# coollabsio/maxio

Hardware: AMD Instinct MI355X
Metric: device-resident RS encode+reconstruct GiB/s (k+m, chunk_size); % HBM roofline (higher is better)
Workload: dtype u8

## Files before the change

maxio_amd/csrc/rs_kernel.hip:

```cpp
#include "kernels.hpp"

#include <cstdlib>

namespace mxec {
namespace {

constexpr int kThreads = 256;
constexpr int fast_vecs(uint32_t r) { return r <= 4 ? 4 : 2; }
constexpr uint64_t kEdgeTile = kThreads * 16;

struct Vec4 {
    uint32_t w[4];
};

__device__ __forceinline__ Vec4 load16(const uint8_t* p) {
    const uint4 v = *reinterpret_cast<const uint4*>(p);
    return Vec4{{v.x, v.y, v.z, v.w}};
}

__device__ __forceinline__ void store16(uint8_t* p, const uint32_t (&w)[4]) {
    *reinterpret_cast<uint4*>(p) = make_uint4(w[0], w[1], w[2], w[3]);
}

__device__ __forceinline__ Vec4 load_partial(const uint8_t* p, int64_t valid, bool aligned) {
    if (aligned && valid >= 16) return load16(p);
    Vec4 r{{0, 0, 0, 0}};
    for (int b = 0; b < 16; ++b)
        if (b < valid) r.w[b >> 2] |= uint32_t(p[b]) << (8 * (b & 3));
    return r;
}

__device__ __forceinline__ void store_partial(uint8_t* p, const uint32_t (&w)[4], int64_t valid,
                                              bool aligned) {
    if (aligned && valid >= 16) {
        store16(p, w);
        return;
    }
    for (int b = 0; b < 16; ++b)
        if (b < valid) p[b] = uint8_t(w[b >> 2] >> (8 * (b & 3)));
}

template <int R>
__device__ __forceinline__ void mac_dword(uint32_t (&acc)[R], uint32_t x, const uint32_t* __restrict__ t,
                                          const uint32_t (&hi)[R][2]) {
    const uint32_t s0 = x & 0x07070707u;
    const uint32_t s1 = (x >> 3) & 0x07070707u;
    const uint32_t s2 = (x >> 6) & 0x03030303u;
#pragma unroll
    for (int i = 0; i < R; ++i) {
        const uint32_t p0 = __builtin_amdgcn_perm(hi[i][0], t[8 * i + 0], s0);
        const uint32_t p1 = __builtin_amdgcn_perm(hi[i][1], t[8 * i + 2], s1);
        const uint32_t p2 = __builtin_amdgcn_perm(s2, t[8 * i + 4], s2);
        acc[i] = __builtin_amdgcn_bitop3_b32(acc[i], p0, p1, 0x96) ^ p2;
    }
}

template <int R, int V>
__device__ __forceinline__ void mac_column(uint32_t (&acc)[V][4][R], const Vec4 (&x)[V],
                                           const uint32_t* __restrict__ t) {
    uint32_t hi[R][2];
#pragma unroll
    for (int i = 0; i < R; ++i) {
        hi[i][0] = __builtin_amdgcn_readfirstlane(t[8 * i + 1]);
        hi[i][1] = __builtin_amdgcn_readfirstlane(t[8 * i + 3]);
        asm volatile("" : "+v"(hi[i][0]), "+v"(hi[i][1]));
    }
#pragma unroll
    for (int v = 0; v < V; ++v)
#pragma unroll
        for (int w = 0; w < 4; ++w) mac_dword<R>(acc[v][w], x[v].w[w], t, hi);
}

template <int R, int V>
__device__ __forceinline__ void mac_column_pair(uint32_t (&acc)[V][4][R], const Vec4 (&xa)[V], const Vec4 (&xb)[V],
                                                const uint32_t* __restrict__ ta, const uint32_t* __restrict__ tb) {
    uint32_t ha[R][2], hb[R][2];
#pragma unroll
    for (int i = 0; i < R; ++i) {
        ha[i][0] = __builtin_amdgcn_readfirstlane(ta[8 * i + 1]);
        ha[i][1] = __builtin_amdgcn_readfirstlane(ta[8 * i + 3]);
        hb[i][0] = __builtin_amdgcn_readfirstlane(tb[8 * i + 1]);
        hb[i][1] = __builtin_amdgcn_readfirstlane(tb[8 * i + 3]);
        asm volatile("" : "+v"(ha[i][0]), "+v"(ha[i][1]), "+v"(hb[i][0]), "+v"(hb[i][1]));
    }
#pragma unroll
    for (int v = 0; v < V; ++v)
#pragma unroll
        for (int w = 0; w < 4; ++w) {
            const uint32_t a = xa[v].w[w], b = xb[v].w[w];
            const uint32_t a0 = a & 0x07070707u, a1 = (a >> 3) & 0x07070707u, a2 = (a >> 6) & 0x03030303u;
            const uint32_t b0 = b & 0x07070707u, b1 = (b >> 3) & 0x07070707u, b2 = (b >> 6) & 0x03030303u;
#pragma unroll
            for (int i = 0; i < R; ++i) {
                const uint32_t pa0 = __builtin_amdgcn_perm(ha[i][0], ta[8 * i + 0], a0);
                const uint32_t pa1 = __builtin_amdgcn_perm(ha[i][1], ta[8 * i + 2], a1);
                const uint32_t pa2 = __builtin_amdgcn_perm(a2, ta[8 * i + 4], a2);
                const uint32_t pb0 = __builtin_amdgcn_perm(hb[i][0], tb[8 * i + 0], b0);
                const uint32_t pb1 = __builtin_amdgcn_perm(hb[i][1], tb[8 * i + 2], b1);
                const uint32_t pb2 = __builtin_amdgcn_perm(b2, tb[8 * i + 4], b2);
                uint32_t t = __builtin_amdgcn_bitop3_b32(acc[v][w][i], pa0, pa1, 0x96);
                t = __builtin_amdgcn_bitop3_b32(t, pa2, pb0, 0x96);
                acc[v][w][i] = __builtin_amdgcn_bitop3_b32(t, pb1, pb2, 0x96);
            }
        }
}

typedef const uint8_t __attribute__((address_space(1)))* gcptr;
typedef uint8_t __attribute__((address_space(1)))* gptr;

typedef uint32_t u32x4 __attribute__((ext_vector_type(4)));

__device__ __forceinline__ Vec4 gload16(gcptr p) {
    const u32x4 v = __builtin_nontemporal_load((const u32x4 __attribute__((address_space(1)))*)(p));
    return Vec4{{v.x, v.y, v.z, v.w}};
}
__device__ __forceinline__ Vec4 gload16_plain(gcptr p) {
    const u32x4 v = *(const u32x4 __attribute__((address_space(1)))*)(p);
    return Vec4{{v.x, v.y, v.z, v.w}};
}
__device__ __forceinline__ void gstore16(gptr p, const uint32_t (&w)[4]) {
    u32x4 v = {w[0], w[1], w[2], w[3]};
    __builtin_nontemporal_store(v, (u32x4 __attribute__((address_space(1)))*)(p));
}

__device__ __forceinline__ Vec4 mask_tail(Vec4 x, int32_t valid) {
#pragma unroll
    for (int w = 0; w < 4; ++w) {
        const int32_t nb = valid - 4 * w;
        const uint32_t mk = nb >= 4 ? 0xFFFFFFFFu : (nb <= 0 ? 0u : (0xFFFFFFFFu >> (32 - 8 * nb)));
        x.w[w] &= mk;
    }
    return x;
}

__device__ __forceinline__ uint32_t any_bits(const uint32_t (&d)[4]) { return d[0] | d[1] | d[2] | d[3]; }

__device__ __forceinline__ void report_first_bad(uint64_t* const* __restrict__ fbp, uint32_t row,
                                                 const uint32_t (&d)[4], uint64_t off) {
    const uint64_t bad = __builtin_amdgcn_ballot_w64(any_bits(d) != 0);
    if (bad == 0) return;
    if ((threadIdx.x & 63u) != uint32_t(__builtin_ctzll(bad))) return;
    const uint32_t w = d[0] ? 0u : d[1] ? 1u : d[2] ? 2u : 3u;
    const uint32_t x = d[0] ? d[0] : d[1] ? d[1] : d[2] ? d[2] : d[3];
    const uint64_t at = off + 4 * w + (uint32_t(__builtin_ctz(x)) >> 3);
    atomicMin(reinterpret_cast<unsigned long long*>(*fbp + row), static_cast<unsigned long long>(at));
}

enum : int { kStore = 0, kCmp = 1, kLocate = 2, kSeed = 3 };

struct LocArgs {
    LocateRec* const* rec = nullptr;
    const uint8_t* field = nullptr;
    const uint8_t* tab = nullptr;
    const uint32_t* off = nullptr;
};

struct LocTally {
    uint32_t first = ~0u;
    uint32_t n = 0;
    uint32_t cmin = ~0u, cmax = 0;
};

template <int R>
__device__ __forceinline__ void locate_dword(LocTally& t, const uint32_t (&d)[R], uint32_t rel, uint64_t col0,
                                             const uint8_t* __restrict__ field, const uint8_t* __restrict__ tab,
                                             const uint64_t* __restrict__ il, uint32_t k) {
    uint32_t any = 0;
#pragma unroll
    for (int i = 0; i < R; ++i) any |= d[i];
    if (any == 0) return;
#pragma unroll 1
    for (uint32_t b = 0; b < 4; ++b) {
        uint32_t s[R], nz = 0;
#pragma unroll
        for (int i = 0; i < R; ++i) {
            s[i] = (d[i] >> (8 * b)) & 0xFFu;
            nz += s[i] != 0;
        }
        if (nz == 0) continue;
        uint32_t c = kLocateNoShard;
        if (nz == 1) {
#pragma unroll
            for (int i = 0; i < R; ++i) c = s[i] ? k + uint32_t(i) : c;
        } else if (nz == uint32_t(R)) {
            if constexpr (R >= 2) {
                const uint32_t l0 = field[s[0]];
                uint32_t dl = uint32_t(field[s[1]]) + 255u - l0;
                dl = dl >= 255u ? dl - 255u : dl;
                const uint32_t j = tab[field[256 + dl]];
                if (j < k) {
                    bool ok = col0 + b < il[j];
#pragma unroll
                    for (int i = 2; i < R; ++i) {
                        uint32_t di = uint32_t(field[s[i]]) + 255u - l0;
                        di = di >= 255u ? di - 255u : di;
                        ok = ok && di == tab[256 * (1 + i) + j];
                    }
                    c = ok ? j : c;
                }
            }
        }
        t.n += 1;
        t.first = min(t.first, rel + b);
        t.cmin = min(t.cmin, c);
        t.cmax = max(t.cmax, c);
    }
}

__device__ __forceinline__ void locate_commit(LocateRec* rec, LocTally t, uint64_t base) {
#pragma unroll
    for (int o = 32; o > 0; o >>= 1) {
        t.first = min(t.first, uint32_t(__shfl_xor(t.first, o)));
        t.n += uint32_t(__shfl_xor(t.n, o));
        t.cmin = min(t.cmin, uint32_t(__shfl_xor(t.cmin, o)));
        t.cmax = max(t.cmax, uint32_t(__shfl_xor(t.cmax, o)));
    }
    if ((threadIdx.x & 63u) != 0 || t.n == 0) return;
    atomicMin(reinterpret_cast<unsigned long long*>(&rec->first_bad), static_cast<unsigned long long>(base + t.first));
    atomicAdd(reinterpret_cast<unsigned long long*>(&rec->n_bad), static_cast<unsigned long long>(t.n));
    atomicMin(&rec->shard_min, t.cmin);
    atomicMax(&rec->shard_max, t.cmax);
}

__global__ void rs_locate_init(LocateRec* __restrict__ recs, uint64_t n) {
    const uint64_t i = uint64_t(blockIdx.x) * blockDim.x + threadIdx.x;
    if (i < n) recs[i] = LocateRec{~uint64_t(0), 0, ~0u, 0};
}

template <int R, int POL = kStore>
__device__ __forceinline__ void edge_step(
    const uint8_t* const* __restrict__ in_ptrs, uint8_t* const* __restrict__ out_ptrs,
    const uint64_t* __restrict__ in_len, const uint64_t* __restrict__ out_len,
    const uint32_t* __restrict__ coef, const uint32_t* __restrict__ coef_off, uint64_t shard_size,
    uint32_t k, uint32_t r_total, uint32_t row0, const uint64_t* __restrict__ edge_list,
    uint32_t steps_per_tile, uint64_t tile_bytes, uint32_t aligned, uint64_t step,
    uint64_t* const* __restrict__ fb_ptrs = nullptr, LocArgs loc = {},
    const uint8_t* const* __restrict__ seed_ptrs = nullptr) {
    const uint64_t e = edge_list[step / steps_per_tile];
    const uint32_t obj = uint32_t(e >> 32);
    const uint64_t col = uint64_t(uint32_t(e)) * tile_bytes + (step % steps_per_tile) * kEdgeTile +
                         threadIdx.x * 16;
    if constexpr (POL == kLocate) {
        if (__builtin_amdgcn_ballot_w64(col < shard_size) == 0) return;
    } else {
        if (col >= shard_size) return;
    }
    const uint32_t* __restrict__ tab = coef + coef_off[obj] + row0 * 8;
    uint32_t acc[1][4][R];
    if constexpr (POL == kSeed) {
#pragma unroll
        for (int i = 0; i < R; ++i) {
            uint64_t olen = out_len[uint64_t(obj) * r_total + row0 + i];
            if (olen > shard_size) olen = shard_size;
            const int64_t valid = col < olen ? int64_t(olen - col) : 0;
            Vec4 sd{{0, 0, 0, 0}};
            if (valid > 0) sd = load_partial(seed_ptrs[uint64_t(obj) * r_total + row0 + i] + col, valid, aligned != 0);
#pragma unroll
            for (int w = 0; w < 4; ++w) acc[0][w][i] = sd.w[w];
        }
    } else {
#pragma unroll
        for (int w = 0; w < 4; ++w)
#pragma unroll
            for (int i = 0; i < R; ++i) acc[0][w][i] = 0;
    }
    const uint8_t* safe = reinterpret_cast<const uint8_t*>(coef);
    auto issue = [&](uint32_t j, Vec4& x, const uint8_t*& p, int64_t& valid) {
        const uint64_t len = in_len[uint64_t(obj) * k + j];
        valid = col < len ? int64_t(len - col) : 0;
        p = in_ptrs[uint64_t(obj) * k + j] + col;
        const bool full = aligned && valid >= 16;
        x = gload16_plain(gcptr(full ? p : safe));
    };
    auto fixup = [&](Vec4& x, const uint8_t* p, int64_t valid) {
        const bool full = aligned && valid >= 16;
#pragma unroll
        for (int w = 0; w < 4; ++w) x.w[w] = full ? x.w[w] : 0u;
        if (valid > 0 && !full) x = load_partial(p, valid, aligned != 0);
    };
    uint32_t j = 0;
    for (; j + 4 <= k; j += 4) {
        Vec4 x[4][1];
        const uint8_t* p[4];
        int64_t valid[4];
#pragma unroll
        for (int u = 0; u < 4; ++u) issue(j + u, x[u][0], p[u], valid[u]);
#pragma unroll
        for (int u = 0; u < 4; ++u) fixup(x[u][0], p[u], valid[u]);
#pragma unroll
        for (int u = 0; u < 4; ++u) mac_column<R, 1>(acc, x[u], tab + (j + u) * r_total * 8);
    }
    for (; j < k; ++j) {
        Vec4 x[1];
        const uint8_t* p;
        int64_t valid;
        issue(j, x[0], p, valid);
        fixup(x[0], p, valid);
        mac_column<R, 1>(acc, x, tab + j * r_total * 8);
    }
    if constexpr (POL == kLocate) {
        uint32_t df[4][R], any = 0;
#pragma unroll
        for (int i = 0; i < R; ++i) {
            uint64_t olen = out_len[uint64_t(obj) * r_total + row0 + i];
            if (olen > shard_size) olen = shard_size;
            const int64_t valid = col < olen ? int64_t(olen - col) : 0;
            Vec4 st{{0, 0, 0, 0}};
            if (valid > 0) st = load_partial(out_ptrs[uint64_t(obj) * r_total + row0 + i] + col, valid, aligned != 0);
            Vec4 d{{acc[0][0][i] ^ st.w[0], acc[0][1][i] ^ st.w[1], acc[0][2][i] ^ st.w[2], acc[0][3][i] ^ st.w[3]}};
            d = mask_tail(d, valid >= 16 ? 16 : int32_t(valid));
#pragma unroll
            for (int w = 0; w < 4; ++w) {
                df[w][i] = d.w[w];
                any |= d.w[w];
            }
        }
        if (__builtin_amdgcn_ballot_w64(any != 0) == 0) return;
        LocTally t;
        const uint8_t* __restrict__ ktab = loc.tab + loc.off[obj];
#pragma unroll
        for (int w = 0; w < 4; ++w)
            locate_dword<R>(t, df[w], threadIdx.x * 16 + 4 * w, col + 4 * w, loc.field, ktab,
                            in_len + uint64_t(obj) * k, k);
        locate_commit(loc.rec[obj], t, col - threadIdx.x * 16);
        return;
    }
    constexpr bool CMP = POL == kCmp;
#pragma unroll
    for (int i = 0; i < R; ++i) {
        uint64_t olen = out_len[uint64_t(obj) * r_total + row0 + i];
        if (olen > shard_size) olen = shard_size;
        if constexpr (CMP) {
            const int64_t valid = col < olen ? int64_t(olen - col) : 0;
            Vec4 st{{0, 0, 0, 0}};
            if (valid > 0) st = load_partial(out_ptrs[uint64_t(obj) * r_total + row0 + i] + col, valid, aligned != 0);
            Vec4 df{{acc[0][0][i] ^ st.w[0], acc[0][1][i] ^ st.w[1], acc[0][2][i] ^ st.w[2], acc[0][3][i] ^ st.w[3]}};
            df = mask_tail(df, valid >= 16 ? 16 : int32_t(valid));
            report_first_bad(fb_ptrs + obj, row0 + i, df.w, col);
        } else if (col < olen) {
            uint32_t o[4] = {acc[0][0][i], acc[0][1][i], acc[0][2][i], acc[0][3][i]};
            store_partial(out_ptrs[uint64_t(obj) * r_total + row0 + i] + col, o, int64_t(olen - col),
                          aligned != 0);
        }
    }
}

template <int R>
__global__ __launch_bounds__(kThreads) void rs_apply_edge(
    const uint8_t* const* __restrict__ in_ptrs, uint8_t* const* __restrict__ out_ptrs,
    const uint64_t* __restrict__ in_len, const uint64_t* __restrict__ out_len,
    const uint32_t* __restrict__ coef, const uint32_t* __restrict__ coef_off, uint64_t shard_size,
    uint32_t k, uint32_t r_total, uint32_t row0, const uint64_t* __restrict__ edge_list,
    uint32_t steps_per_tile, uint64_t tile_bytes, uint32_t aligned, uint64_t n_steps) {
    for (uint64_t step = blockIdx.x; step < n_steps; step += gridDim.x)
        edge_step<R>(in_ptrs, out_ptrs, in_len, out_len, coef, coef_off, shard_size, k, r_total, row0, edge_list,
                     steps_per_tile, tile_bytes, aligned, step);
}

template <int R>
__global__ __launch_bounds__(kThreads) void rs_verify_edge(
    const uint8_t* const* __restrict__ in_ptrs, uint8_t* const* __restrict__ out_ptrs,
    const uint64_t* __restrict__ in_len, const uint64_t* __restrict__ out_len,
    const uint32_t* __restrict__ coef, const uint32_t* __restrict__ coef_off, uint64_t shard_size,
    uint32_t k, uint32_t r_total, uint32_t row0, const uint64_t* __restrict__ edge_list,
    uint32_t steps_per_tile, uint64_t tile_bytes, uint32_t aligned, uint64_t n_steps,
    uint64_t* const* __restrict__ fb_ptrs) {
    for (uint64_t step = blockIdx.x; step < n_steps; step += gridDim.x)
        edge_step<R, kCmp>(in_ptrs, out_ptrs, in_len, out_len, coef, coef_off, shard_size, k, r_total, row0,
                           edge_list, steps_per_tile, tile_bytes, aligned, step, fb_ptrs);
}

template <int R>
__global__ __launch_bounds__(kThreads) void rs_update_edge(
    const uint8_t* const* __restrict__ in_ptrs, uint8_t* const* __restrict__ out_ptrs,
    const uint64_t* __restrict__ in_len, const uint64_t* __restrict__ out_len,
    const uint32_t* __restrict__ coef, const uint32_t* __restrict__ coef_off, uint64_t shard_size,
    uint32_t k, uint32_t r_total, uint32_t row0, const uint64_t* __restrict__ edge_list,
    uint32_t steps_per_tile, uint64_t tile_bytes, uint32_t aligned, uint64_t n_steps,
    const uint8_t* const* __restrict__ seed_ptrs) {
    for (uint64_t step = blockIdx.x; step < n_steps; step += gridDim.x)
        edge_step<R, kSeed>(in_ptrs, out_ptrs, in_len, out_len, coef, coef_off, shard_size, k, r_total, row0,
                            edge_list, steps_per_tile, tile_bytes, aligned, step, nullptr, {}, seed_ptrs);
}

template <int R>
__global__ __launch_bounds__(kThreads) void rs_locate_edge(
    const uint8_t* const* __restrict__ in_ptrs, uint8_t* const* __restrict__ out_ptrs,
    const uint64_t* __restrict__ in_len, const uint64_t* __restrict__ out_len,
    const uint32_t* __restrict__ coef, const uint32_t* __restrict__ coef_off, uint64_t shard_size,
    uint32_t k, uint32_t r_total, uint32_t row0, const uint64_t* __restrict__ edge_list,
    uint32_t steps_per_tile, uint64_t tile_bytes, uint32_t aligned, uint64_t n_steps, LocArgs loc) {
    for (uint64_t step = blockIdx.x; step < n_steps; step += gridDim.x)
        edge_step<R, kLocate>(in_ptrs, out_ptrs, in_len, out_len, coef, coef_off, shard_size, k, r_total, row0,
                              edge_list, steps_per_tile, tile_bytes, aligned, step, nullptr, loc);
}

__device__ __forceinline__ Vec4 gload16_upto(gcptr p, int32_t valid, gcptr safe) {
    return mask_tail(gload16(valid > 0 ? p : safe), valid);
}

template <int R, int V, int POL = kStore>
__device__ __forceinline__ void rs_tile(const uint8_t* const* __restrict__ ip, const uint64_t* __restrict__ il,
                                        uint8_t* const* __restrict__ op, const uint64_t* __restrict__ ol,
                                        const uint32_t* __restrict__ tab, uint32_t k, uint32_t stride,
                                        uint64_t base, gcptr safe, uint64_t* const* __restrict__ fbp = nullptr,
                                        uint32_t row = 0, LocArgs loc = {},
                                        const uint8_t* const* __restrict__ sp = nullptr) {
    constexpr bool CMP = POL == kCmp || POL == kLocate;
    constexpr uint32_t kTile = kThreads * 16 * V;
    const uint64_t end = base + kTile;
    const uint64_t lane = base + threadIdx.x * 16;
    const int32_t lane_off = int32_t(threadIdx.x * 16);

    uint32_t acc[V][4][R];
    if constexpr (POL == kSeed) {
#pragma unroll
        for (int i = 0; i < R; ++i) {
            const uint64_t olen = ol[i];
            gcptr q = ((gcptr)(sp[i])) + lane;
            Vec4 sd[V];
            if (olen >= end) {
#pragma unroll
                for (int v = 0; v < V; ++v) sd[v] = gload16(q + v * kThreads * 16);
            } else if (olen <= base) {
#pragma unroll
                for (int v = 0; v < V; ++v) sd[v] = Vec4{{0, 0, 0, 0}};
            } else {
                const int32_t d = int32_t(olen - base) - lane_off;
#pragma unroll
                for (int v = 0; v < V; ++v)
                    sd[v] = gload16_upto(q + v * kThreads * 16, d - v * int32_t(kThreads * 16), safe);
            }
#pragma unroll
            for (int v = 0; v < V; ++v)
#pragma unroll
                for (int w = 0; w < 4; ++w) acc[v][w][i] = sd[v].w[w];
        }
    } else {
#pragma unroll
        for (int v = 0; v < V; ++v)
#pragma unroll
            for (int w = 0; w < 4; ++w)
#pragma unroll
                for (int i = 0; i < R; ++i) acc[v][w][i] = 0;
    }

    auto load_in = [&](uint32_t jj, Vec4 (&x)[V]) {
        const uint64_t len = il[jj];
        gcptr p = ((gcptr)(ip[jj])) + lane;
        if (len >= end) {
#pragma unroll
            for (int v = 0; v < V; ++v) x[v] = gload16(p + v * kThreads * 16);
        } else if (len <= base) {
#pragma unroll
            for (int v = 0; v < V; ++v) x[v] = Vec4{{0, 0, 0, 0}};
        } else {
            const int32_t d = int32_t(len - base) - lane_off;
#pragma unroll
            for (int v = 0; v < V; ++v)
                x[v] = gload16_upto(p + v * kThreads * 16, d - v * int32_t(kThreads * 16), safe);
        }
    };

    uint32_t j = 0;
    for (; j + 4 <= k; j += 4) {
        Vec4 x[4][V];
        if (il[j] >= end && il[j + 1] >= end && il[j + 2] >= end && il[j + 3] >= end) {
#pragma unroll
            for (int jj = 0; jj < 4; ++jj) {
                gcptr p = ((gcptr)(ip[j + jj])) + lane;
#pragma unroll
                for (int v = 0; v < V; ++v) x[jj][v] = gload16(p + v * kThreads * 16);
            }
        } else {
#pragma unroll
            for (int jj = 0; jj < 4; ++jj) load_in(j + jj, x[jj]);
        }
        if constexpr (R >= 3) {
            mac_column_pair<R, V>(acc, x[0], x[1], tab + (j + 0) * stride * 8, tab + (j + 1) * stride * 8);
            mac_column_pair<R, V>(acc, x[2], x[3], tab + (j + 2) * stride * 8, tab + (j + 3) * stride * 8);
        } else {
#pragma unroll
            for (int jj = 0; jj < 4; ++jj) mac_column<R, V>(acc, x[jj], tab + (j + jj) * stride * 8);
        }
    }
    for (; j < k; ++j) {
        if (il[j] <= base) continue;
        Vec4 x[V];
        load_in(j, x);
        mac_column<R, V>(acc, x, tab + j * stride * 8);
    }
    if constexpr (CMP) {
        Vec4 st[R][V];
#pragma unroll
        for (int i = 0; i < R; ++i) {
            const uint64_t olen = ol[i];
            gcptr o = ((gcptr)(op[i])) + lane;
            if (olen >= end) {
#pragma unroll
                for (int v = 0; v < V; ++v) st[i][v] = gload16(o + v * kThreads * 16);
            } else if (olen <= base) {
#pragma unroll
                for (int v = 0; v < V; ++v)
#pragma unroll
                    for (int w = 0; w < 4; ++w) st[i][v].w[w] = acc[v][w][i];
            } else {
                const int32_t d = int32_t(olen - base) - lane_off;
#pragma unroll
                for (int v = 0; v < V; ++v) {
                    const int32_t valid = d - v * int32_t(kThreads * 16);
                    st[i][v] = gload16(valid > 0 ? o + v * kThreads * 16 : safe);
                    if (valid < 16) {
                        Vec4 a{{acc[v][0][i], acc[v][1][i], acc[v][2][i], acc[v][3][i]}};
                        const Vec4 keep = mask_tail(Vec4{{~0u, ~0u, ~0u, ~0u}}, valid);
#pragma unroll
                        for (int w = 0; w < 4; ++w) st[i][v].w[w] = (st[i][v].w[w] & keep.w[w]) | (a.w[w] & ~keep.w[w]);
                    }
                }
            }
        }
        if constexpr (POL == kLocate) {
            uint32_t any = 0;
#pragma unroll
            for (int i = 0; i < R; ++i)
#pragma unroll
                for (int v = 0; v < V; ++v)
#pragma unroll
                    for (int w = 0; w < 4; ++w) {
                        acc[v][w][i] ^= st[i][v].w[w];
                        any |= acc[v][w][i];
                    }
            if (__builtin_amdgcn_ballot_w64(any != 0) == 0) return;
            LocTally t;
            const uint8_t* __restrict__ ktab = loc.tab + *loc.off;
#pragma unroll
            for (int v = 0; v < V; ++v)
#pragma unroll
                for (int w = 0; w < 4; ++w) {
                    const uint32_t rel = uint32_t(lane_off) + uint32_t(v) * kThreads * 16 + 4 * w;
                    locate_dword<R>(t, acc[v][w], rel, base + rel, loc.field, ktab, il, k);
                }
            locate_commit(*loc.rec, t, base);
            return;
        }
#pragma unroll
        for (int i = 0; i < R; ++i) {
            uint32_t df[V][4], any = 0;
#pragma unroll
            for (int v = 0; v < V; ++v)
#pragma unroll
                for (int w = 0; w < 4; ++w) {
                    df[v][w] = acc[v][w][i] ^ st[i][v].w[w];
                    any |= df[v][w];
                }
            if (__builtin_amdgcn_ballot_w64(any != 0) == 0) continue;
#pragma unroll
            for (int v = 0; v < V; ++v) {
                if (__builtin_amdgcn_ballot_w64(any_bits(df[v]) != 0) == 0) continue;
                report_first_bad(fbp, row + uint32_t(i), df[v], lane + uint64_t(v) * kThreads * 16);
                break;
            }
        }
        return;
    }
#pragma unroll
    for (int i = 0; i < R; ++i) {
        const uint64_t olen = ol[i];
        if (olen <= base) continue;
        gptr o = ((gptr)(op[i])) + lane;
        const int32_t d = olen >= end ? int32_t(kTile) : int32_t(olen - base) - lane_off;
#pragma unroll
        for (int v = 0; v < V; ++v) {
            uint32_t ov[4] = {acc[v][0][i], acc[v][1][i], acc[v][2][i], acc[v][3][i]};
            if (olen >= end) {
                gstore16(o + v * kThreads * 16, ov);
            } else {
                const int32_t valid = d - v * int32_t(kThreads * 16);
                if (valid >= 16) {
                    gstore16(o + v * kThreads * 16, ov);
                } else if (valid > 0) {
                    for (int b = 0; b < valid; ++b)
                        o[v * kThreads * 16 + b] = uint8_t(ov[b >> 2] >> (8 * (b & 3)));
                }
            }
        }
    }
}

template <int R, int V, bool GRP, int POL>
__device__ __forceinline__ void fast_tiles(
    const uint8_t* const* __restrict__ in_ptrs, uint8_t* const* __restrict__ out_ptrs,
    const uint64_t* __restrict__ in_len, const uint64_t* __restrict__ out_len,
    const uint32_t* __restrict__ coef, const uint32_t* __restrict__ coef_off, uint32_t k_uniform,
    uint32_t r_total, uint32_t row0, uint32_t tiles_per_obj, uint64_t n_tiles,
    const RsTileRec* __restrict__ tiles, uint64_t* const* __restrict__ fb_ptrs, LocArgs loc = {},
    const uint8_t* const* __restrict__ seed_ptrs = nullptr) {
    constexpr uint32_t kTile = kThreads * 16 * V;
    const gcptr safe = (gcptr)(reinterpret_cast<const uint8_t*>(coef));
    RsTileRec next{};
    if constexpr (GRP) next = tiles[blockIdx.x];
    for (uint64_t tile = blockIdx.x; tile < n_tiles; tile += gridDim.x) {
        uint32_t obj, k;
        uint64_t base, in0;
        if constexpr (GRP) {
            const RsTileRec cur = next;
            if (tile + gridDim.x < n_tiles) next = tiles[tile + gridDim.x];
            obj = cur.obj;
            k = cur.k;
            in0 = cur.in0;
            base = uint64_t(cur.local) * kTile;
        } else {
            obj = uint32_t(tile / tiles_per_obj);
            base = (tile - uint64_t(obj) * tiles_per_obj) * kTile;
            k = k_uniform;
            in0 = uint64_t(obj) * k;
        }
        LocArgs lo = loc;
        if constexpr (POL == kLocate) {
            lo.rec = loc.rec + obj;
            lo.off = loc.off + obj;
        }
        rs_tile<R, V, POL>(in_ptrs + in0, in_len + in0, out_ptrs + uint64_t(obj) * r_total + row0,
                           out_len + uint64_t(obj) * r_total + row0, coef + coef_off[obj] + row0 * 8, k, r_total, base,
                           safe, POL == kCmp ? fb_ptrs + obj : nullptr, row0, lo,
                           POL == kSeed ? seed_ptrs + uint64_t(obj) * r_total + row0 : nullptr);
    }
}

template <int R, int V, bool GRP>
__global__ __launch_bounds__(kThreads) void rs_apply_fast(
    const uint8_t* const* __restrict__ in_ptrs, uint8_t* const* __restrict__ out_ptrs,
    const uint64_t* __restrict__ in_len, const uint64_t* __restrict__ out_len,
    const uint32_t* __restrict__ coef, const uint32_t* __restrict__ coef_off, uint32_t k_uniform,
    uint32_t r_total, uint32_t row0, uint32_t tiles_per_obj, uint64_t n_tiles,
    const RsTileRec* __restrict__ tiles) {
    fast_tiles<R, V, GRP, kStore>(in_ptrs, out_ptrs, in_len, out_len, coef, coef_off, k_uniform, r_total, row0,
                                  tiles_per_obj, n_tiles, tiles, nullptr);
}

template <int R, int V, bool GRP>
__global__ __launch_bounds__(kThreads) void rs_verify_fast(
    const uint8_t* const* __restrict__ in_ptrs, uint8_t* const* __restrict__ out_ptrs,
    const uint64_t* __restrict__ in_len, const uint64_t* __restrict__ out_len,
    const uint32_t* __restrict__ coef, const uint32_t* __restrict__ coef_off, uint32_t k_uniform,
    uint32_t r_total, uint32_t row0, uint32_t tiles_per_obj, uint64_t n_tiles,
    const RsTileRec* __restrict__ tiles, uint64_t* const* __restrict__ fb_ptrs) {
    fast_tiles<R, V, GRP, kCmp>(in_ptrs, out_ptrs, in_len, out_len, coef, coef_off, k_uniform, r_total, row0,
                                tiles_per_obj, n_tiles, tiles, fb_ptrs);
}

template <int R, int V>
__global__ __launch_bounds__(kThreads) void rs_update_fast(
    const uint8_t* const* __restrict__ in_ptrs, uint8_t* const* __restrict__ out_ptrs,
    const uint64_t* __restrict__ in_len, const uint64_t* __restrict__ out_len,
    const uint32_t* __restrict__ coef, const uint32_t* __restrict__ coef_off, uint32_t k_uniform,
    uint32_t r_total, uint32_t row0, uint32_t tiles_per_obj, uint64_t n_tiles,
    const uint8_t* const* __restrict__ seed_ptrs) {
    fast_tiles<R, V, false, kSeed>(in_ptrs, out_ptrs, in_len, out_len, coef, coef_off, k_uniform, r_total, row0,
                                   tiles_per_obj, n_tiles, nullptr, nullptr, {}, seed_ptrs);
}

template <int R, int V, bool GRP>
__global__ __launch_bounds__(kThreads) void rs_locate_fast(
    const uint8_t* const* __restrict__ in_ptrs, uint8_t* const* __restrict__ out_ptrs,
    const uint64_t* __restrict__ in_len, const uint64_t* __restrict__ out_len,
    const uint32_t* __restrict__ coef, const uint32_t* __restrict__ coef_off, uint32_t k_uniform,
    uint32_t r_total, uint32_t row0, uint32_t tiles_per_obj, uint64_t n_tiles,
    const RsTileRec* __restrict__ tiles, LocArgs loc) {
    fast_tiles<R, V, GRP, kLocate>(in_ptrs, out_ptrs, in_len, out_len, coef, coef_off, k_uniform, r_total, row0,
                                   tiles_per_obj, n_tiles, tiles, nullptr, loc);
}

__global__ __launch_bounds__(kThreads) void rs_apply_multi(
    const uint8_t* const* __restrict__ in_ptrs, uint8_t* const* __restrict__ out_ptrs,
    const uint64_t* __restrict__ in_len, const uint64_t* __restrict__ out_len,
    const uint32_t* __restrict__ coef, const uint32_t* __restrict__ coef_off, uint64_t n_tiles,
    const RsTileRec* __restrict__ tiles) {
    constexpr int V = fast_vecs(kMultiR);
    constexpr uint32_t kTile = kThreads * 16 * V;
    const gcptr safe = (gcptr)(reinterpret_cast<const uint8_t*>(coef));
    RsTileRec next = tiles[blockIdx.x];
    for (uint64_t tile = blockIdx.x; tile < n_tiles; tile += gridDim.x) {
        const RsTileRec cur = next;
        if (tile + gridDim.x < n_tiles) next = tiles[tile + gridDim.x];
        const uint32_t k = cur.k & 0xFFFFu, r = (cur.k >> 16) & 0xFFu;
        const uint64_t base = uint64_t(cur.local) * kTile;
        const uint8_t* const* ip = in_ptrs + cur.in0;
        const uint64_t* il = in_len + cur.in0;
        uint8_t* const* op = out_ptrs + uint64_t(cur.obj) * kMultiR;
        const uint64_t* ol = out_len + uint64_t(cur.obj) * kMultiR;
        const uint32_t* tab = coef + coef_off[cur.obj];
        switch (r) {
            case 1: rs_tile<1, V>(ip, il, op, ol, tab, k, 1, base, safe); break;
            case 2: rs_tile<2, V>(ip, il, op, ol, tab, k, 2, base, safe); break;
            case 3: rs_tile<3, V>(ip, il, op, ol, tab, k, 3, base, safe); break;
            default: rs_tile<4, V>(ip, il, op, ol, tab, k, 4, base, safe); break;
        }
    }
}

uint64_t grid_of(const RsArgs& a, int n_cus, int per_cu, uint64_t n) {
    uint64_t blocks = uint64_t(n_cus) * uint64_t(per_cu);
    if (a.max_blocks && blocks > a.max_blocks) blocks = a.max_blocks;
    return blocks > n ? n : blocks;
}

LocArgs loc_args(const RsArgs& a) { return LocArgs{a.locate, a.loc_field, a.loc_tab, a.loc_off}; }

template <int R, int V, bool GRP>
hipError_t launch_fast(const RsArgs& a, uint32_t tiles_per_obj, uint64_t n_tiles, uint64_t blocks,
                       hipStream_t s) {
    if (a.seed_ptrs) {
        if constexpr (!GRP) {
            if (a.first_bad) return hipErrorInvalidValue;
            hipLaunchKernelGGL((rs_update_fast<R, V>), dim3(uint32_t(blocks)), dim3(kThreads), 0, s, a.in_ptrs,
                               a.out_ptrs, a.in_len, a.out_len, a.coef, a.coef_off, a.k, a.r_total, a.row0,
                               tiles_per_obj, n_tiles, a.seed_ptrs);
            return hipGetLastError();
        }
        return hipErrorInvalidValue;
    }
    if (a.first_bad)
        hipLaunchKernelGGL((rs_verify_fast<R, V, GRP>), dim3(uint32_t(blocks)), dim3(kThreads), 0, s, a.in_ptrs,
                           a.out_ptrs, a.in_len, a.out_len, a.coef, a.coef_off, a.k, a.r_total, a.row0,
                           tiles_per_obj, n_tiles, a.tiles, a.first_bad);
    else
        hipLaunchKernelGGL((rs_apply_fast<R, V, GRP>), dim3(uint32_t(blocks)), dim3(kThreads), 0, s, a.in_ptrs,
                           a.out_ptrs, a.in_len, a.out_len, a.coef, a.coef_off, a.k, a.r_total, a.row0,
                           tiles_per_obj, n_tiles, a.tiles);
    return hipGetLastError();
}

template <int R, bool GRP>
hipError_t launch_locate(const RsArgs& a, uint32_t tiles_per_obj, uint64_t n_tiles, uint64_t blocks,
                         hipStream_t s) {
    if constexpr (R >= 2) {
        if (a.row0 != 0 || a.r != a.r_total) return hipErrorInvalidValue;
        hipLaunchKernelGGL((rs_locate_fast<R, fast_vecs(R), GRP>), dim3(uint32_t(blocks)), dim3(kThreads), 0, s,
                           a.in_ptrs, a.out_ptrs, a.in_len, a.out_len, a.coef, a.coef_off, a.k, a.r_total, a.row0,
                           tiles_per_obj, n_tiles, a.tiles, loc_args(a));
        return hipGetLastError();
    }
    return hipErrorInvalidValue;
}

hipError_t launch_multi(const RsArgs& a, int n_cus, hipStream_t s) {
    const RsVariant v = rs_group_variant(kMultiR);
    const uint64_t blocks = grid_of(a, n_cus, v.blocks_per_cu, a.n_tiles);
    hipLaunchKernelGGL(rs_apply_multi, dim3(uint32_t(blocks)), dim3(kThreads), 0, s, a.in_ptrs, a.out_ptrs, a.in_len,
                       a.out_len, a.coef, a.coef_off, a.n_tiles, a.tiles);
    return hipGetLastError();
}

template <int R>
hipError_t launch_grouped(const RsArgs& a, int n_cus, hipStream_t s) {
    const uint64_t blocks = grid_of(a, n_cus, rs_group_variant(uint32_t(R)).blocks_per_cu, a.n_tiles);
    if (a.locate) return launch_locate<R, true>(a, 0, a.n_tiles, blocks, s);
    return launch_fast<R, fast_vecs(R), true>(a, 0, a.n_tiles, blocks, s);
}

template <int R>
hipError_t launch_r(const RsArgs& a, int n_cus, hipStream_t s, const RsVariant& var) {
    const uint64_t tile = rs_tile_bytes(var);
    if (a.seed_ptrs && (a.locate || a.first_bad)) return hipErrorInvalidValue;
    if (a.aligned) {
        const uint32_t tiles_per_obj = uint32_t((a.shard_size + tile - 1) / tile);
        const uint64_t n_tiles = uint64_t(tiles_per_obj) * a.n_obj;
        const uint64_t blocks = grid_of(a, n_cus, var.blocks_per_cu, n_tiles);
        constexpr int V = fast_vecs(R);
        if (a.locate && var.vecs == V) return launch_locate<R, false>(a, tiles_per_obj, n_tiles, blocks, s);
        if (!a.locate && var.vecs == V) return launch_fast<R, V, false>(a, tiles_per_obj, n_tiles, blocks, s);
        if (!a.locate && var.vecs == 2) return launch_fast<R, 2, false>(a, tiles_per_obj, n_tiles, blocks, s);
        return hipErrorInvalidValue;
    }
    if (a.n_edge && a.edge_tile_bytes != tile) return hipErrorInvalidValue;
    if (a.n_edge) {
        const uint32_t steps = uint32_t(tile / kEdgeTile);
        const uint64_t n_steps = a.n_edge * steps;
        const uint64_t blocks = grid_of(a, n_cus, 8, n_steps);
        if (a.locate) {
            if constexpr (R >= 2) {
                if (a.row0 != 0 || a.r != a.r_total) return hipErrorInvalidValue;
                hipLaunchKernelGGL((rs_locate_edge<R>), dim3(uint32_t(blocks)), dim3(kThreads), 0, s,
                                   a.in_ptrs, a.out_ptrs, a.in_len, a.out_len, a.coef, a.coef_off,
                                   a.shard_size, a.k, a.r_total, a.row0, a.edge_list, steps, tile, a.aligned,
                                   n_steps, loc_args(a));
                return hipGetLastError();
            }
            return hipErrorInvalidValue;
        }
        if (a.first_bad) {
            hipLaunchKernelGGL((rs_verify_edge<R>), dim3(uint32_t(blocks)), dim3(kThreads), 0, s,
                               a.in_ptrs, a.out_ptrs, a.in_len, a.out_len, a.coef, a.coef_off,
                               a.shard_size, a.k, a.r_total, a.row0, a.edge_list, steps, tile, a.aligned,
                               n_steps, a.first_bad);
            return hipGetLastError();
        }
        if (a.seed_ptrs) {
            hipLaunchKernelGGL((rs_update_edge<R>), dim3(uint32_t(blocks)), dim3(kThreads), 0, s,
                               a.in_ptrs, a.out_ptrs, a.in_len, a.out_len, a.coef, a.coef_off,
                               a.shard_size, a.k, a.r_total, a.row0, a.edge_list, steps, tile, a.aligned,
                               n_steps, a.seed_ptrs);
            return hipGetLastError();
        }
        hipLaunchKernelGGL((rs_apply_edge<R>), dim3(uint32_t(blocks)), dim3(kThreads), 0, s,
                           a.in_ptrs, a.out_ptrs, a.in_len, a.out_len, a.coef, a.coef_off,
                           a.shard_size, a.k, a.r_total, a.row0, a.edge_list, steps, tile, a.aligned,
                           n_steps);
        return hipGetLastError();
    }
    return hipSuccess;
}

}

uint64_t rs_tile_bytes(const RsVariant& v) { return uint64_t(kThreads) * 16 * uint64_t(v.vecs); }

RsVariant rs_default_variant(uint32_t r_total) {
    RsVariant v;
    v.vecs = fast_vecs(r_total);
    v.blocks_per_cu = r_total <= 2 ? 1024 : 512;
#ifdef MXEC_LAB
    if (const char* e = getenv("MXEC_RS_BPC")) {
        const int b = atoi(e);
        if (b > 0 && b <= 4096) v.blocks_per_cu = b;
    }
#endif
    return v;
}

RsVariant rs_group_variant(uint32_t r) {
    RsVariant v = rs_default_variant(r);
    v.blocks_per_cu = 512;
#ifdef MXEC_LAB
    static const int env_b = [] {
        const char* e = getenv("MXEC_RS_GROUP_BPC");
        return e ? atoi(e) : 0;
    }();
    if (env_b > 0 && env_b <= 4096) v.blocks_per_cu = env_b;
#endif
    return v;
}

hipError_t launch_rs_apply_variant(const RsArgs& a, int n_cus, hipStream_t s, const RsVariant& v) {
    switch (a.r) {
        case 1: return launch_r<1>(a, n_cus, s, v);
        case 2: return launch_r<2>(a, n_cus, s, v);
        case 3: return launch_r<3>(a, n_cus, s, v);
        case 4: return launch_r<4>(a, n_cus, s, v);
        case 5: return launch_r<5>(a, n_cus, s, v);
        case 6: return launch_r<6>(a, n_cus, s, v);
        case 7: return launch_r<7>(a, n_cus, s, v);
        case 8: return launch_r<8>(a, n_cus, s, v);
        default: return hipErrorInvalidValue;
    }
}

hipError_t launch_locate_init(LocateRec* recs, uint64_t n, hipStream_t s) {
    if (n == 0) return hipSuccess;
    if (n > (uint64_t(1) << 31)) return hipErrorInvalidValue;
    hipLaunchKernelGGL(rs_locate_init, dim3(uint32_t((n + kThreads - 1) / kThreads)), dim3(kThreads), 0, s, recs, n);
    return hipGetLastError();
}

hipError_t launch_rs_apply(const RsArgs& a, int n_cus, hipStream_t s) {
    if (a.tiles && a.seed_ptrs) return hipErrorInvalidValue;
    if (a.tiles && a.multi) {
        if (!a.aligned || a.row0 != 0 || a.first_bad || a.locate) return hipErrorInvalidValue;
        if (a.n_tiles == 0) return hipSuccess;
        return launch_multi(a, n_cus, s);
    }
    if (a.tiles) {
        if (!a.aligned || a.row0 != 0 || a.r != a.r_total) return hipErrorInvalidValue;
        if (a.n_tiles == 0) return hipSuccess;
        switch (a.r) {
            case 1: return launch_grouped<1>(a, n_cus, s);
            case 2: return launch_grouped<2>(a, n_cus, s);
            case 3: return launch_grouped<3>(a, n_cus, s);
            case 4: return launch_grouped<4>(a, n_cus, s);
            case 5: return launch_grouped<5>(a, n_cus, s);
            case 6: return launch_grouped<6>(a, n_cus, s);
            case 7: return launch_grouped<7>(a, n_cus, s);
            case 8: return launch_grouped<8>(a, n_cus, s);
            default: return hipErrorInvalidValue;
        }
    }
    RsVariant v = rs_default_variant(a.r_total);
    if (a.blocks_per_cu) v.blocks_per_cu = int(a.blocks_per_cu);
    return launch_rs_apply_variant(a, n_cus, s, v);
}

}
```

Baseline: 3837.

## Compact live input columns and batch edge-tile loads before a single wait

Rewrites the k-loop's slow path, used for ragged-length inputs, so that columns whose length is at or below the tile base are compacted out. Up to four live columns are then loaded together with predicated loads that redirect out-of-range lanes to a safe pointer, followed by mask_tail and one explicit vmcnt(0) wait. The separate scalar remainder loop is folded in, and MACs are dispatched on the live count, so dead columns skip their table MACs. The aim is to overlap the memory latency of edge tiles and cut per-column branching. The cost is more complex selection logic and an explicit full wait that may serialize memory traffic.

```diff
diff --git a/maxio_amd/csrc/rs_kernel.hip b/maxio_amd/csrc/rs_kernel.hip
--- a/maxio_amd/csrc/rs_kernel.hip
+++ b/maxio_amd/csrc/rs_kernel.hip
@@ -8,6 +8,7 @@
 constexpr int kThreads = 256;
 constexpr int fast_vecs(uint32_t r) { return r <= 4 ? 4 : 2; }
 constexpr uint64_t kEdgeTile = kThreads * 16;
+constexpr int kWaitVm0 = 0x0F70;
 
 struct Vec4 {
     uint32_t w[4];
@@ -445,27 +446,11 @@
                 for (int i = 0; i < R; ++i) acc[v][w][i] = 0;
     }
 
-    auto load_in = [&](uint32_t jj, Vec4 (&x)[V]) {
-        const uint64_t len = il[jj];
-        gcptr p = ((gcptr)(ip[jj])) + lane;
-        if (len >= end) {
-#pragma unroll
-            for (int v = 0; v < V; ++v) x[v] = gload16(p + v * kThreads * 16);
-        } else if (len <= base) {
-#pragma unroll
-            for (int v = 0; v < V; ++v) x[v] = Vec4{{0, 0, 0, 0}};
-        } else {
-            const int32_t d = int32_t(len - base) - lane_off;
-#pragma unroll
-            for (int v = 0; v < V; ++v)
-                x[v] = gload16_upto(p + v * kThreads * 16, d - v * int32_t(kThreads * 16), safe);
-        }
-    };
-
-    uint32_t j = 0;
-    for (; j + 4 <= k; j += 4) {
+    for (uint32_t j = 0; j < k; j += 4) {
         Vec4 x[4][V];
-        if (il[j] >= end && il[j + 1] >= end && il[j + 2] >= end && il[j + 3] >= end) {
+        uint32_t sl[4] = {j, j + 1, j + 2, j + 3}, n = 4;
+        const uint32_t cnt = k - j < 4 ? k - j : 4;
+        if (cnt == 4 && il[j] >= end && il[j + 1] >= end && il[j + 2] >= end && il[j + 3] >= end) {
 #pragma unroll
             for (int jj = 0; jj < 4; ++jj) {
                 gcptr p = ((gcptr)(ip[j + jj])) + lane;
@@ -473,22 +458,59 @@
                 for (int v = 0; v < V; ++v) x[jj][v] = gload16(p + v * kThreads * 16);
             }
         } else {
-#pragma unroll
-            for (int jj = 0; jj < 4; ++jj) load_in(j + jj, x[jj]);
-        }
+            n = 0;
+            sl[0] = sl[1] = sl[2] = sl[3] = j;
+#pragma unroll
+            for (uint32_t u = 0; u < 4; ++u) {
+                const uint32_t jj = j + (u < cnt ? u : cnt - 1);
+                const bool live = u < cnt && il[jj] > base;
+#pragma unroll
+                for (uint32_t q = 0; q < 4; ++q) sl[q] = live && n == q ? jj : sl[q];
+                n += live ? 1u : 0u;
+            }
+            const bool lone = n == 1;
+            sl[2] = lone ? sl[0] : sl[2];
+#pragma unroll
+            for (uint32_t q = 0; q < 4; ++q) {
+                const bool on = lone ? q == 2 : q < n;
+                if (on) {
+                    const uint64_t len = il[sl[q]];
+                    gcptr p = ((gcptr)(ip[sl[q]])) + lane;
+                    const int32_t d = (len >= end ? int32_t(kTile) : int32_t(len - base)) - lane_off;
+#pragma unroll
+                    for (int v = 0; v < V; ++v)
+                        x[q][v] = gload16(d - v * int32_t(kThreads * 16) > 0 ? p + v * kThreads * 16 : safe);
+                } else {
+#pragma unroll
+                    for (int v = 0; v < V; ++v) x[q][v] = Vec4{{0, 0, 0, 0}};
+                }
+            }
+#pragma unroll
+            for (uint32_t q = 0; q < 4; ++q) {
+                const bool on = lone ? q == 2 : q < n;
+                const uint64_t len = on ? il[sl[q]] : end;
+                if (len < end) {
+                    const int32_t d = int32_t(len - base) - lane_off;
+#pragma unroll
+                    for (int v = 0; v < V; ++v) x[q][v] = mask_tail(x[q][v], d - v * int32_t(kThreads * 16));
+                }
+            }
+            __builtin_amdgcn_s_waitcnt(kWaitVm0);
+        }
+        const uint32_t* t0 = tab + sl[0] * stride * 8;
+        const uint32_t* t1 = tab + sl[1] * stride * 8;
+        const uint32_t* t2 = tab + sl[2] * stride * 8;
+        const uint32_t* t3 = tab + sl[3] * stride * 8;
         if constexpr (R >= 3) {
-            mac_column_pair<R, V>(acc, x[0], x[1], tab + (j + 0) * stride * 8, tab + (j + 1) * stride * 8);
-            mac_column_pair<R, V>(acc, x[2], x[3], tab + (j + 2) * stride * 8, tab + (j + 3) * stride * 8);
+            if (n >= 2) mac_column_pair<R, V>(acc, x[0], x[1], t0, t1);
+            if (n == 4) mac_column_pair<R, V>(acc, x[2], x[3], t2, t3);
+            if (n & 1) mac_column<R, V>(acc, x[2], t2);
         } else {
-#pragma unroll
-            for (int jj = 0; jj < 4; ++jj) mac_column<R, V>(acc, x[jj], tab + (j + jj) * stride * 8);
-        }
-    }
-    for (; j < k; ++j) {
-        if (il[j] <= base) continue;
-        Vec4 x[V];
-        load_in(j, x);
-        mac_column<R, V>(acc, x, tab + j * stride * 8);
+            if (n >= 2) mac_column<R, V>(acc, x[0], t0);
+            if (n >= 2) mac_column<R, V>(acc, x[1], t1);
+            if (n >= 3 || n == 1) mac_column<R, V>(acc, x[2], t2);
+            if (n == 4) mac_column<R, V>(acc, x[3], t3);
+        }
     }
     if constexpr (CMP) {
         Vec4 st[R][V];
```

After: 3842, median of 4. About the same (+0.1%).
